# jdhuang-csm/hybrid-drt

Measured on AMD Instinct MI355X. Metric: DRT fits/sec (256 freq x 512 tau, batched), higher is better.
Workload: dtype f64

## Files before the change

hybrid-drt_amd/_ffi.py:

```python
from __future__ import annotations

import ctypes as C
import os
import sys
import threading

import numpy as np

_HERE = os.path.dirname(os.path.abspath(__file__))
LIB_PATH = os.environ.get("HIPDRT_LIB", os.path.join(_HERE, "libhipdrt.so"))

MODE_INTERP, MODE_TRAPZ = 0, 1
RESPONSE_POT, RESPONSE_EXPDECAY = 0, 1
QP_OPTIMAL, QP_MAXITER, QP_SINGULAR_LATE, QP_SINGULAR, QP_ABORTED = 0, 1, 2, -1, -2


class HipDrtError(RuntimeError):
    pass


class QpOpts(C.Structure):
    _fields_ = [("abstol", C.c_double), ("reltol", C.c_double), ("feastol", C.c_double), ("maxiters", C.c_int)]


# ... 44 lines not shown
    "hipdrt_impedance_lookup": [_vp, C.c_double, C.c_int, C.c_int, _dp, _dp, _dp, _dp],
    "hipdrt_impedance_matrix": [_vp, C.c_int, C.c_int, _dp, C.c_int, _dp, C.c_int, C.c_int, C.c_int, C.c_double,
                                C.c_int, _dp, _dp, _dp, _dp, C.c_int, _dp, _dp],
    "hipdrt_impedance_matrix_dev": [_vp, C.c_int, C.c_int, _dp, C.c_int, _dp, C.c_int, C.c_int, C.c_int, C.c_double,
                                    C.c_int, _dp, _dp, _dp, _dp, C.c_int, _vp, _vp, C.c_int, C.POINTER(C.c_float)],
    "hipdrt_phasor_z_matrix": [_vp, _dp, C.c_int, _dp, C.c_int, C.c_double, _dp, _dp],
    "hipdrt_phasor_v_matrix": [_vp, _dp, C.c_int, _dp, C.c_int, C.c_double, _dp, _dp, C.c_int, _dp, _dp],
    "hipdrt_chrono_var_matrix": [_vp, _dp, C.c_int, _ip, C.c_int, C.c_double, C.c_int, _dp],
    "hipdrt_response_lookup": [_vp, C.c_double, C.c_int, C.c_int, _dp, _dp],
    "hipdrt_response_matrix": [_vp, _dp, C.c_int, _dp, C.c_int, _dp, _dp, C.c_int, C.c_int, C.c_double, C.c_int, _dp, _dp,
                               C.c_int, _dp, _dp],
    "hipdrt_plan_bytes_per_spectrum": [C.c_int, C.c_int, C.c_int, C.POINTER(C.c_longlong)],
    "hipdrt_response_matrix_variant": [_vp, _dp, C.c_int, _dp, C.c_int, _dp, _dp, _dp, C.c_int, C.c_int, C.c_double, C.c_int,
                                       _dp, _dp],
    "hipdrt_nonuniform_gaussian_filter1d": [_vp, _dp, C.c_int, _dp, _ip, C.c_int, _ip, _dp, C.c_int, _dp, _dp, C.c_longlong,
                                            _ip, _ip, _dp],
    "hipdrt_penalty_matrices": [_vp, _dp, C.c_int, C.c_double, C.c_int, _dp, _dp, _dp],
    "hipdrt_eis_var_matrix": [_vp, _dp, C.c_int, C.c_double, C.c_double, C.c_int, _dp],
    "hipdrt_qp_batch": [_vp, C.c_int, C.c_int, C.c_int, _dp, _dp, C.c_int, _dp, C.POINTER(QpOpts), _dp, _ip, _dp, _ip],
    "hipdrt_qp_profile": [_vp, C.POINTER(C.c_ulonglong), C.c_int, C.c_int],
    "hipdrt_debug_qp_occupancy": [_vp, C.c_int, C.c_int],
    "hipdrt_debug_qp_group": [_vp, C.c_int],
    "hipdrt_debug_exact_zero_shortcuts": [_vp, C.c_int],
    "hipdrt_debug_qp_waves": [_vp, C.c_int],
    "hipdrt_debug_stream_pool": [_vp, C.c_int, C.POINTER(C.c_void_p), _ip, _ip, _ip],
    "hipdrt_comm_unique_id": [C.c_char_p],
    "hipdrt_comm_create": [C.c_int, C.c_int, C.c_int, C.c_char_p, C.POINTER(_vp)],
    "hipdrt_comm_destroy": [_vp],
    "hipdrt_comm_info": [_vp, _ip, _ip, _ip],
    "hipdrt_comm_broadcast_dev": [_vp, _vp, C.c_longlong, C.c_int],
    "hipdrt_comm_gather_dev": [_vp, _vp, C.c_longlong, _vp, C.c_int],
    "hipdrt_comm_broadcast": [_vp, _dp, C.c_longlong, C.c_int],
    "hipdrt_comm_gather": [_vp, _dp, C.c_longlong, _dp, C.c_int],
    "hipdrt_comm_allreduce_max": [_vp, _dp],
    "hipdrt_comm_barrier": [_vp],
    "hipdrt_device_alloc": [_vp, C.c_longlong, C.POINTER(_vp)],
    "hipdrt_device_free": [_vp, _vp],
    "hipdrt_device_synchronize": [_vp],
    "hipdrt_device_probe": [C.c_int],
    "hipdrt_weighted_gram": [_vp, C.c_int, C.c_int, C.c_int, _dp, _dp, _dp, C.c_int, _dp, _dp, _dp, _dp],
    "hipdrt_default_fit_opts": [C.POINTER(FitOpts)],
    "hipdrt_plan_create": [_vp, _dp, C.c_int, _dp, C.c_int, C.c_double, C.c_int, C.c_int, C.c_int, C.c_int, C.c_int,
                           _dp, _dp, _dp, _dp, C.POINTER(FitOpts), C.c_int, C.POINTER(_vp)],
    "hipdrt_plan_create_prepared": [_vp, C.POINTER(PreparedDesc), _dp, _dp, _dp, _dp, _dp, _dp, _dp, C.POINTER(FitOpts),
                                    C.c_int, C.POINTER(_vp)],
    "hipdrt_plan_upload_prepared": [_vp, C.c_int, C.c_int, _dp, _dp],
# ... 299 lines not shown
        _check(self._lib.hipdrt_device_free(self._h, _vp(ptr)))

    def device_synchronize(self):
        _check(self._lib.hipdrt_device_synchronize(self._h))

    def debug_qp_group(self, members):
        _check(self._lib.hipdrt_debug_qp_group(self._h, int(members)))
        self._qp_group_override = int(members)

    def debug_qp_waves(self, waves):
        _check(self._lib.hipdrt_debug_qp_waves(self._h, int(waves)))

    def debug_stream_pool(self):
        size = C.c_int(0)
        _check(self._lib.hipdrt_debug_stream_pool(self._h, 0, None, None, None, C.byref(size)))
        n = size.value
        st, ho, ru = (C.c_void_p * n)(), (C.c_int * n)(), (C.c_int * n)()
        _check(self._lib.hipdrt_debug_stream_pool(self._h, n, st, ho, ru, C.byref(size)))
        return [st[i] for i in range(n)], [ho[i] for i in range(n)], [ru[i] for i in range(n)]

    def debug_exact_zero_shortcuts(self, on):
        _check(self._lib.hipdrt_debug_exact_zero_shortcuts(self._h, int(bool(on))))

    def qp_profile(self, reset=True):
        buf = (C.c_ulonglong * 64)()
        _check(self._lib.hipdrt_qp_profile(self._h, buf, 64, int(reset)))
        return [int(v) for v in buf]

    def qp_timeline(self):
        n = 64 + 8 * 16 * 8
        buf = (C.c_ulonglong * n)()
        _check(self._lib.hipdrt_qp_profile(self._h, buf, n, 0))
        return np.array(buf[64:], dtype=np.uint64).reshape(8, 16, 8)

    def qp_timeline_mean(self, reset=True):
        nt = 8 * 16 * 8
        n = 64 + 2 * nt + 1
        buf = (C.c_ulonglong * n)()
        _check(self._lib.hipdrt_qp_profile(self._h, buf, n, int(reset)))
        cnt = int(buf[64 + 2 * nt])
        return np.array(buf[64 + nt:64 + 2 * nt], dtype=np.float64).reshape(8, 16, 8) / max(cnt, 1), cnt

    def weighted_gram(self, A, w, b, l2=None, l1=None):
        A, w, b = _f64(A), _f64(w), _f64(b)
        if w.ndim == 1:
            w, b = w[None, :], b[None, :]
# ... 322 lines not shown
```

hybrid-drt_amd/csrc/api.hip:

```cpp
#include <algorithm>
#include <chrono>
#include <cmath>
#include <cstdlib>
#include <cstring>
#include <functional>
#include <memory>
#include <mutex>
#include <new>
#include <stdexcept>

#include "common.hpp"
#include <thread>
#include <vector>

namespace hipdrt {
static thread_local std::string g_err;
void set_error(const std::string& msg) { g_err = msg; }
}

using namespace hipdrt;

struct hipdrt_plan {
    hipdrt_ctx* ctx = nullptr;
    int nf = 0, ntau = 0, n = 0, m = 0, ns = 0, ngrid = 0, ny = 0, mode = 0, toeplitz_a = 0, toeplitz_m = 0;
// ... 246 lines not shown
    hipError_t e = hipGetDeviceCount(&count);
    if (e != hipSuccess || count <= 0) {
        set_error("no HIP device visible (libhipdrt has no CPU fallback)");
        return HIPDRT_E_NODEVICE;
    }
    HIPDRT_REQUIRE(device >= 0 && device < count, "device index out of range");
    HIPDRT_CHECK(hipSetDevice(device)); (void)hipGetLastError();
    hipDeviceProp_t prop;
    HIPDRT_CHECK(hipGetDeviceProperties(&prop, device));
    std::string arch = prop.gcnArchName;
    if (arch.rfind("gfx950", 0) != 0) {
        set_error("device " + std::to_string(device) + " is " + arch + "; libhipdrt is built for gfx950 only");
        return HIPDRT_E_NODEVICE;
    }
    auto* c = new hipdrt_ctx();
    c->device = device;
    c->num_cu = prop.multiProcessorCount;
    c->hbm_bytes = prop.totalGlobalMem;
    c->arch = arch.substr(0, arch.find(':'));
    if (const char* wv = std::getenv("HIPDRT_QP_WAVES")) {
        const int w = std::atoi(wv);
        if (w == 4 || w == 8) c->qp_waves = w;
    }
    if (!pool_hold(c)) { delete c; set_error("no HIP stream could be created on device " + std::to_string(device)); return HIPDRT_E_HIP; }
    *out = c;
    return HIPDRT_OK;
} HIPDRT_CATCH

static std::mutex g_life;

static void free_ctx(hipdrt_ctx* ctx) {
    pool_drop(ctx);
    delete ctx;
}

int hipdrt_destroy(hipdrt_ctx* ctx) try {
    if (!ctx) return HIPDRT_OK;
    std::lock_guard<std::mutex> lk(g_life);
    if (ctx->plans > 0) { ctx->released = true; return HIPDRT_OK; }
    free_ctx(ctx);
    return HIPDRT_OK;
} HIPDRT_CATCH

void* hipdrt_stream(hipdrt_ctx* ctx) { return ctx ? (void*)ctx->stream : nullptr; }

int hipdrt_synchronize(hipdrt_ctx* ctx) try {
// ... 380 lines not shown
    std::lock_guard<std::mutex> lock(pl->mu);
    *size = (int)pl->st.size();
    for (int i = 0; i < std::min(cap, *size); ++i) {
        if (streams) streams[i] = pl->st[i];
        if (holders) holders[i] = pl->holders[i];
        if (running) running[i] = pl->running[i];
    }
    return HIPDRT_OK;
} HIPDRT_CATCH

int hipdrt_debug_qp_waves(hipdrt_ctx* ctx, int waves) try {
    HIPDRT_REQUIRE(ctx, "NULL pointer");
    HIPDRT_REQUIRE(waves == -1 || waves == 4 || waves == 8, "waves: 4, 8 or -1");
    ctx->qp_waves = waves;
    return HIPDRT_OK;
} HIPDRT_CATCH

int hipdrt_debug_exact_zero_shortcuts(hipdrt_ctx* ctx, int on) try {
    HIPDRT_REQUIRE(ctx, "NULL pointer");
    ctx->zero_shortcuts = on ? 1 : 0;
    return HIPDRT_OK;
} HIPDRT_CATCH

int hipdrt_debug_qp_occupancy(hipdrt_ctx* ctx, int threads, int n) try {
    if (!ctx || hipSetDevice(ctx->device) != hipSuccess) return -1;
    return qp_occupancy(threads, n);
} HIPDRT_CATCH

int hipdrt_qp_profile(hipdrt_ctx* ctx, unsigned long long* cycles, int n, int reset) try {
    HIPDRT_REQUIRE(ctx && cycles, "NULL pointer");
    HIPDRT_CHECK(hipSetDevice(ctx->device)); (void)hipGetLastError();
    HIPDRT_CHECK(hipStreamSynchronize(ctx->stream));
    return qp_profile_read(cycles, n, reset) < 0 ? HIPDRT_E_HIP : HIPDRT_OK;
} HIPDRT_CATCH

int hipdrt_weighted_gram(hipdrt_ctx* ctx, int B, int m, int n, const double* A, const double* w, const double* b,
                         int l2_batched, const double* l2, const double* l1, double* P, double* q) try {
    HIPDRT_REQUIRE(ctx && A && w && b && P && q, "NULL pointer");
    HIPDRT_REQUIRE(B >= 1 && m >= 1 && n >= 1, "B, m, n >= 1");
    HIPDRT_CHECK(hipSetDevice(ctx->device)); (void)hipGetLastError();
    hipStream_t st = ctx->stream;
    DevBuf dA, dw, db, dl2, dl1, dP, dq;
    TRY(upload(dA, A, (size_t)m * n * sizeof(double), st));
    TRY(upload(dw, w, (size_t)B * m * sizeof(double), st));
    TRY(upload(db, b, (size_t)B * m * sizeof(double), st));
    if (l2) TRY(upload(dl2, l2, (size_t)(l2_batched ? B : 1) * n * n * sizeof(double), st));
    if (l1) TRY(upload(dl1, l1, (size_t)n * sizeof(double), st));
    HIPDRT_CHECK(dP.alloc((size_t)B * n * n * sizeof(double)));
    HIPDRT_CHECK(dq.alloc((size_t)B * n * sizeof(double)));
    launch_weighted_gram(st, B, m, n, dA.d(), n, dw.d(), db.d(), l2 ? dl2.d() : nullptr,
                         l2_batched ? (long long)n * n : 0, n, l1 ? dl1.d() : nullptr, dP.d(), n, (long long)n * n,
                         dq.d(), nullptr);
    LAUNCH_OK();
    HIPDRT_CHECK(hipMemcpyAsync(P, dP.p, (size_t)B * n * n * sizeof(double), hipMemcpyDeviceToHost, st));
    HIPDRT_CHECK(hipMemcpyAsync(q, dq.p, (size_t)B * n * sizeof(double), hipMemcpyDeviceToHost, st));
    HIPDRT_CHECK(hipStreamSynchronize(st));
    return HIPDRT_OK;
} HIPDRT_CATCH


void hipdrt_default_fit_opts(hipdrt_fit_opts* o) {
    if (!o) return;
    std::memset(o, 0, sizeof(*o));
    o->rp_scale = 14;
    const double dw[3] = {1.5, 1.0, 0.5}, sd[3] = {1, 1000, 1000}, sa[3] = {5, 10, 25}, ra[3] = {0.15, 0.2, 0.25};
    for (int k = 0; k < 3; ++k) {
        o->derivative_weights[k] = dw[k]; o->sigma_ds[k] = sd[k]; o->s_alpha[k] = sa[k]; o->s_0[k] = 1.0;
        o->rho_alpha[k] = ra[k]; o->rho_0[k] = 1.0;
    }
    o->l1_lambda_0 = 0; o->l2_lambda_0 = 142;
    o->iw_l1_lambda_0 = 1e-4; o->iw_l2_lambda_0 = 1e-4;
    o->ohmic_penalty = 1e-6; o->inductance_penalty = 1e-6; o->inductance_scale = 1e-5;
    o->eis_vmm_epsilon = 0.25; o->eis_reim_cor = 0.25;
    o->xtol = 1e-2; o->max_iter = 50; o->nonneg = 1; o->scale_data = 1; o->fit_ohmic = 1; o->fit_inductance = 1;
    o->update_scale = 0; o->eff_hp = 1;
// ... 277 lines not shown
} HIPDRT_CATCH

int hipdrt_plan_upload(hipdrt_plan* p, int B, const double* z_re, const double* z_im) try {
    HIPDRT_REQUIRE(p && z_re && z_im, "NULL pointer");
    HIPDRT_REQUIRE(!p->prepared, "prepared plans take hipdrt_plan_upload_prepared");
    HIPDRT_REQUIRE(B >= 1 && B <= p->capacity, "1 <= B <= capacity");
    HIPDRT_CHECK(hipSetDevice(p->ctx->device)); (void)hipGetLastError();
    hipStream_t st = p->ctx->stream;
    const size_t bytes = (size_t)B * p->nf * sizeof(double);
    HIPDRT_CHECK(hipMemcpyAsync(p->z_re.p, z_re, bytes, hipMemcpyHostToDevice, st));
    HIPDRT_CHECK(hipMemcpyAsync(p->z_im.p, z_im, bytes, hipMemcpyHostToDevice, st));
    HIPDRT_CHECK(hipStreamSynchronize(st));
    p->B = B;
    return HIPDRT_OK;
} HIPDRT_CATCH

static GramL2 plan_l2(const hipdrt_plan* p, double l2_lambda_0, const double* derivative_weights, double dop_l2_lambda_0) {
    GramL2 g{};
    g.l2 = nullptr; g.ldm = p->ldm; g.ns = p->ns; g.use_rho = 1;
    g.sym = p->prepared ? 0 : p->toeplitz_m;
    g.toep = p->toeplitz_m;
    g.toep_maxd = (p->toeplitz_m && !(p->ctx && !p->ctx->zero_shortcuts)) ? p->toep_maxd : -1;
    g.spec_zero = p->spec_zero;
    for (int k = 0; k < 3; ++k) { g.mk[k] = p->mk[k].d(); g.dfac[k] = l2_lambda_0 * derivative_weights[k]; }
    g.s = p->s.d(); g.rho = p->rho.d();
    if (p->prepared && p->desc.dop_size > 0) {
        g.dop_start = p->desc.dop_start; g.dop_size = p->desc.dop_size; g.dop_rho = p->dop_rho.d();
        for (int k = 0; k < 3; ++k) g.dop_dfac[k] = dop_l2_lambda_0 * p->desc.dop_derivative_weights[k];
    }
    return g;
}

struct FinalP { GramL2 g; const double* w; };
static FinalP plan_final_p(const hipdrt_plan* p, int b) {
    FinalP f{plan_l2(p, p->opts.l2_lambda_0, p->opts.derivative_weights, p->prepared ? p->desc.dop_l2_lambda_0 : 0.0),
             p->has_weight_factors() ? p->w_eff.d() : p->w.d()};
    if (b >= 0) {
        f.g.s += (size_t)b * 3 * p->n; f.g.rho += (size_t)b * 3;
        if (f.g.dop_size > 0) f.g.dop_rho += (size_t)b * 3;
        f.w += (size_t)b * p->m;
    }
    return f;
}

static int plan_toep_reach(hipdrt_plan* p) {
    p->toep_maxd = -1;
// ... 221 lines not shown
            launch_scale_rows(st, B, m, p->w.d(), nullptr, 0, p->weight_factor, nullptr, p->w.d());
            launch_scale_rows(st, B, m, p->w.d(), p->wrow.d(), p->wrow_batched, 1.0, nullptr, p->w_eff.d());
        }
        wfin = p->w_eff.d();
    }
    return outer_finish(p, st, tm, wfin);
}

static int subbatch_count(const hipdrt_plan* p) {
    if (p->prepared || p->hist_b >= 0 || p->has_weight_factors() || p->opts.outlier_p > 0.0 || p->qp_G != 0) return 1;
    const int k_auto = p->B >= 1000 ? std::min(4, pool_size(p->ctx->device)) : (p->B >= 600 ? 2 : 1);
    int k = p->subbatches >= 1 ? std::min(p->subbatches, std::max(1, p->B / 64)) : k_auto;
    const int force = p->ctx ? p->ctx->qp_force_group : -1;
    if (qp_group_size(p->B, p->n, force) != 0) return 1;
    while (k > 1 && qp_group_size(p->B / k, p->n, force) != 0) --k;
    return k;
}

static int make_view(hipdrt_plan* p, hipdrt_subfit& sf, int idx, int b0, int nb) {
    hipdrt_plan& v = sf.view;
    sf.ctx.device = p->ctx->device; sf.ctx.num_cu = p->ctx->num_cu; sf.ctx.hbm_bytes = p->ctx->hbm_bytes; sf.ctx.arch = p->ctx->arch;
    sf.ctx.qp_force_group = p->ctx->qp_force_group;
    sf.ctx.zero_shortcuts = p->ctx->zero_shortcuts;
    sf.ctx.qp_waves = p->ctx->qp_waves;
    v.ctx = &sf.ctx;
    v.nf = p->nf; v.ntau = p->ntau; v.n = p->n; v.m = p->m; v.ns = p->ns; v.ngrid = p->ngrid; v.ny = p->ny; v.mode = p->mode;
    v.toeplitz_a = p->toeplitz_a; v.toeplitz_m = p->toeplitz_m; v.toep_maxd = p->toep_maxd; v.spec_zero = p->spec_zero; v.idx_rinf = p->idx_rinf; v.idx_induc = p->idx_induc;
    v.ldrm = p->ldrm; v.ldm = p->ldm; v.ldp = p->ldp; v.ldl = p->ldl; v.eps = p->eps; v.opts = p->opts;
    v.capacity = nb; v.B = nb; v.qp_G = p->qp_G; v.subbatches = 1;
    auto whole = [](DevBuf& d, const DevBuf& s_) { d.alias(s_, 0, s_.bytes); };
    whole(v.freq, p->freq); whole(v.tau, p->tau); whole(v.ln_tau, p->ln_tau); whole(v.wt_re, p->wt_re); whole(v.wt_im, p->wt_im);
    whole(v.lut6, p->lut6); whole(v.a_re, p->a_re); whole(v.a_im, p->a_im); whole(v.cr, p->cr); whole(v.rm, p->rm);
    for (int k = 0; k < 3; ++k) whole(v.mk[k], p->mk[k]);
    whole(v.vmm, p->vmm); whole(v.h, p->h); whole(v.l1, p->l1); whole(v.h_init, p->h_init); whole(v.vmm_base, p->vmm_base);
    whole(v.Ptmp, p->Ptmp);
    const SpecDims d = spec_dims(p);
    for (const PerSpectrumBuf& e : kPerSpectrum) {
        const size_t per = e.bytes(d);
        (v.*e.buf).alias(p->*e.buf, (size_t)b0 * per, (size_t)nb * per);
    }
    v.n_active.alias(p->n_active_sub, (size_t)idx * sizeof(int), sizeof(int));
    return HIPDRT_OK;
}

int hipdrt_plan_bytes_per_spectrum(int nf, int ntau, int ns, long long* bytes) try {
    HIPDRT_REQUIRE(bytes && nf >= 1 && ntau >= 1 && ns >= 0, "arguments");
// ... 443 lines not shown
```

hybrid-drt_amd/csrc/common.hpp:

```cpp
#pragma once
#include <hip/hip_runtime.h>

#include <cstdio>
#include <string>
#include <vector>

#include "../../include/hipdrt.h"
#include "../../include/hipdrt_debug.h"

namespace hipdrt {

void set_error(const std::string& msg);

#define HIPDRT_CHECK(expr)                                                                     \
    do {                                                                                       \
        hipError_t _e = (expr);                                                                \
        if (_e != hipSuccess) {                                                                \
            hipdrt::set_error(std::string(#expr) + ": " + hipGetErrorString(_e) + " (" +       \
                              __FILE__ + ":" + std::to_string(__LINE__) + ")");                \
            return HIPDRT_E_HIP;                                                               \
        }                                                                                      \
    } while (0)

#define HIPDRT_REQUIRE(cond, msg)                                                              \
// ... 40 lines not shown

inline int round_up(int v, int m) { return (v + m - 1) / m * m; }

inline int set_lds_limit(const void* f, size_t bytes, const char* what) {
    const hipError_t e = hipFuncSetAttribute(f, hipFuncAttributeMaxDynamicSharedMemorySize, (int)bytes);
    if (e != hipSuccess) { set_error(std::string("hipFuncSetAttribute(") + what + "): " + hipGetErrorString(e)); return HIPDRT_E_HIP; }
    return HIPDRT_OK;
}

}

struct hipdrt_ctx {
    int device = 0;
    hipStream_t stream = nullptr;
    int pool_idx = -1;
    int num_cu = 0;
    size_t hbm_bytes = 0;
    std::string arch;
    int plans = 0;
    bool released = false;
    int qp_force_group = -1;
    int zero_shortcuts = 1;
    int qp_waves = -1;
};

namespace hipdrt {

void ensure_stream_pool(int device);

void launch_lookup(hipStream_t st, double eps, int ngrid, int ny, const double* wt_re, const double* wt_im,
                   double* z_re, double* z_im);
void launch_lookup_slopes(hipStream_t st, int ngrid, const double* xp, const double* fp, double* slopes);
void launch_impedance_matrix(hipStream_t st, int B, int freq_batched, const double* freq, int nf, const double* tau,
                             int ntau, int mode, int toeplitz, double eps, int ngrid, const double* lut6, int ny,
                             double* a_re, double* a_im, double* cr_scratch);
void launch_phasor_z(hipStream_t st, const double* freq, int nf, const double* nu, int nnu, double eps, double* zre,
                     double* zim);
void launch_phasor_v(hipStream_t st, const double* times, int nt, const double* nu, int nnu, double eps,
                     const double* step_times, const double* step_sizes, int nsteps, double* rm, double* layered);
void launch_chrono_vmm(hipStream_t st, const double* tt, int nt, const int* seg, int nseg, double eps, int uniform,
                       double* vmm);
void launch_response_lookup(hipStream_t st, double eps, int ngrid, int ny, const double* td, double* v);
void launch_response_matrix(hipStream_t st, const double* times, int nt, const double* tau, int ntau,
                            const double* step_times, const double* step_sizes, int nsteps, int mode, double eps,
                            int ngrid, const double* lut3, int ny, double* a, double* layered);
void launch_response_variant(hipStream_t st, const double* times, int nt, const double* tau, int ntau,
// ... 5 lines not shown
void launch_penalty(hipStream_t st, const double* ln_tau, int n, double eps, int toeplitz, double* m0, double* m1,
                    double* m2, int ld, int pad);
void launch_eis_vmm(hipStream_t st, const double* freq, int nf, double vmm_eps, double reim_cor, int uniform,
                    double* vmm);

struct GramL2 {
    const double* l2;
    long long l2_stride;
    int ldl2;
    const double* mk[3];
    int ldm;
    const double* s;
    const double* rho;
    double dfac[3];
    int ns;
    int use_rho;
    int sym;
    int toep;
    int toep_maxd;
    int spec_zero;
    int dop_start, dop_size;
    const double* dop_rho;
    double dop_dfac[3];
};
void launch_gram_l2(hipStream_t st, int B, int m, int n, const double* A, int lda, const double* w, const GramL2& g,
                    double* P, int ldp, long long p_stride, const int* active, double* Ppk = nullptr,
                    long long ppk_stride = 0, int nchp = 0, long long a_stride = 0);
void launch_pack_p(hipStream_t st, int B, int n, const double* P, int ldp, long long p_stride, double* Ppk,
                   long long ppk_stride, int nchp);
inline int qp_nchp(int n) { return round_up(n, 32) / 16; }
inline size_t qp_ppk_doubles(int n) { return (size_t)qp_nchp(n) * qp_nchp(n) * 256; }
void launch_qvec_batched(hipStream_t s, int B, int m, int n, const double* rm, int ldrm, const double* w, const double* y,
                         const double* l1, double l1_scalar, double* q, const int* active);
void launch_qvec(hipStream_t st, int B, int m, int n, const double* A, int lda, const double* w, const double* y,
                 const double* l1, double l1_scalar, double* q, const int* active, long long a_stride = 0);
void launch_weighted_gram(hipStream_t st, int B, int m, int n, const double* A, int lda, const double* w,
                          const double* b, const double* l2, long long l2_stride, int ldl2, const double* l1,
                          double* P, int ldp, long long p_stride, double* q, const int* active);

struct FitState {
    int nf, m, n, ns, ldrm, ldm;
    int toeplitz_m;
    int toep_reach;
    int continue_mode;
    int min_iter;
    double basis_area;
    hipdrt_fit_opts opts;
    int prepared;
    hipdrt_prepared_desc desc;
    long long rm_stride;
    double* rm_rw;
    const double* vz_strength;
    const double* vz_entry;
    double *dop_rho, *dop_xmx;
    double* outlier_t;
    double* hist_dop_rho;
    const double* rm;
    const double* vmm;
    const double* vmm_iw;
    const double* mk[3];
    const double *z_re, *z_im;
// ... 83 lines not shown
```

hybrid-drt_amd/csrc/gram.hip:

```cpp
#include "common.hpp"

namespace hipdrt {

typedef double v4d __attribute__((ext_vector_type(4)));

static constexpr int GT = 64;
static constexpr int GK = 16;
static constexpr int GLD = 80;


template <bool DOP, bool ROWP>
__global__ __launch_bounds__(256, 5) void gram_kernel(int m, int n, const double* __restrict__ A, int lda,
                                                   const double* __restrict__ w, GramL2 g, double* __restrict__ P,
                                                   int ldp, long long p_stride, const int* __restrict__ active,
                                                   int ntile, double* __restrict__ Ppk, long long ppk_stride, int nchp,
                                                   long long a_stride) {
    const int b = blockIdx.y;
    if (active && !active[b]) return;
    A += (size_t)b * a_stride;
    int t = blockIdx.x, ti = 0;
    while (t >= ti + 1) { t -= ti + 1; ++ti; }
    const int tj = t;
    const int i0 = ti * GT, j0 = tj * GT;
    const bool diag = (ti == tj);

    __shared__ double sI[GK * GLD];
    __shared__ double sJ[GK * GLD];

    const int tid = threadIdx.x, lane = tid & 63, wv = tid >> 6;
    const int wi = (wv >> 1) * 32, wj = (wv & 1) * 32;
    const double* wb = w + (size_t)b * m;

    v4d acc[2][2];
#pragma unroll
    for (int a = 0; a < 2; ++a)
#pragma unroll
        for (int c = 0; c < 2; ++c) acc[a][c] = (v4d){0.0, 0.0, 0.0, 0.0};

    const int sk = tid >> 4, sc = (tid & 15) * 4;
    const bool vec2 = ((lda | n) & 1) == 0;
    double vi[4], vj[4], wkr = 0.0;
    auto fetch = [&](int k0) {
        const int k = k0 + sk;
#pragma unroll
        for (int e = 0; e < 4; ++e) { vi[e] = 0.0; vj[e] = 0.0; }
        wkr = 0.0;
        if (k < m) {
            wkr = wb[k];
            const double* row = A + (size_t)k * lda;
            if (vec2) {
#pragma unroll
                for (int e = 0; e < 4; e += 2) {
                    const int ci = i0 + sc + e, cj = j0 + sc + e;
                    if (ci < n) { const double2 t = *reinterpret_cast<const double2*>(row + ci); vi[e] = t.x; vi[e + 1] = t.y; }
                    if (!diag && cj < n) { const double2 t = *reinterpret_cast<const double2*>(row + cj); vj[e] = t.x; vj[e + 1] = t.y; }
                }
            } else {
#pragma unroll
                for (int e = 0; e < 4; ++e) {
                    const int ci = i0 + sc + e, cj = j0 + sc + e;
                    if (ci < n) vi[e] = row[ci];
                    if (!diag && cj < n) vj[e] = row[cj];
                }
            }
        }
    };
    const int nt16 = (n + 15) >> 4;
    const int tr0 = __builtin_amdgcn_readfirstlane((i0 + wi) >> 4), tc0 = __builtin_amdgcn_readfirstlane((j0 + wj) >> 4);
    const bool need00 = tr0 < nt16 && tc0 < nt16 && tr0 >= tc0;
    const bool need01 = tr0 < nt16 && tc0 + 1 < nt16 && tr0 >= tc0 + 1;
    const bool need10 = tr0 + 1 < nt16 && tc0 < nt16 && tr0 + 1 >= tc0;
    const bool need11 = tr0 + 1 < nt16 && tc0 + 1 < nt16 && tr0 + 1 >= tc0 + 1;
    fetch(0);
    for (int k0 = 0; k0 < m; k0 += GK) {
        __syncthreads();
        *reinterpret_cast<double2*>(&sI[sk * GLD + sc]) = make_double2(wkr * vi[0], wkr * vi[1]);
        *reinterpret_cast<double2*>(&sI[sk * GLD + sc + 2]) = make_double2(wkr * vi[2], wkr * vi[3]);
        if (!diag) {
            *reinterpret_cast<double2*>(&sJ[sk * GLD + sc]) = make_double2(wkr * vj[0], wkr * vj[1]);
            *reinterpret_cast<double2*>(&sJ[sk * GLD + sc + 2]) = make_double2(wkr * vj[2], wkr * vj[3]);
        }
        __syncthreads();
        if (k0 + GK < m) fetch(k0 + GK);
        const double* sj = diag ? sI : sJ;
#pragma unroll
        for (int kk = 0; kk < GK; kk += 4) {
            const int kr = kk + (lane >> 4);
            double a0 = sI[kr * GLD + wi + (lane & 15)];
            double a1 = sI[kr * GLD + wi + 16 + (lane & 15)];
            double b0 = sj[kr * GLD + wj + (lane & 15)];
            double b1 = sj[kr * GLD + wj + 16 + (lane & 15)];
            if (need00) acc[0][0] = __builtin_amdgcn_mfma_f64_16x16x4f64(b0, a0, acc[0][0], 0, 0, 0);
            if (need01) acc[0][1] = __builtin_amdgcn_mfma_f64_16x16x4f64(b1, a0, acc[0][1], 0, 0, 0);
            if (need10) acc[1][0] = __builtin_amdgcn_mfma_f64_16x16x4f64(b0, a1, acc[1][0], 0, 0, 0);
            if (need11) acc[1][1] = __builtin_amdgcn_mfma_f64_16x16x4f64(b1, a1, acc[1][1], 0, 0, 0);
        }
    }

    double (*sqI)[GT] = reinterpret_cast<double (*)[GT]>(sI);
    double (*sqJ)[GT] = reinterpret_cast<double (*)[GT]>(sJ);
    constexpr int TW = 2 * GT;
    double (*tw)[TW] = reinterpret_cast<double (*)[TW]>(sI + 3 * GT);
    const int dbase = i0 - j0 - (GT - 1);
    double fac[3] = {0, 0, 0};
    const bool l2on = g.s && !(!DOP && g.toep && g.toep_maxd >= 0 && (j0 >= g.ns || g.spec_zero) && i0 >= g.ns && dbase > g.toep_maxd);
    if (l2on) {
#pragma unroll
        for (int k = 0; k < 3; ++k) fac[k] = g.dfac[k] * (g.use_rho ? g.rho[(size_t)b * 3 + k] : 1.0);
        __syncthreads();
        const double* sb_ = g.s + (size_t)b * 3 * n;
        for (int e = tid; e < 3 * GT; e += 256) {
            const int k = e / GT, c = e % GT;
            sqI[k][c] = (i0 + c < n) ? sqrt(sb_[k * n + i0 + c]) : 0.0;
            sqJ[k][c] = (j0 + c < n) ? sqrt(sb_[k * n + j0 + c]) : 0.0;
        }
        if (g.toep) {
            const int nd = n - g.ns;
            for (int e = tid; e < 3 * TW; e += 256) {
                const int k = e / TW, sl = e % TW;
                int dd = dbase + sl;
                dd = dd < 0 ? -dd : dd;
                tw[k][sl] = (g.dfac[k] > 0.0 && dd < nd) ? g.mk[k][(size_t)g.ns * g.ldm + g.ns + dd] * fac[k] : 0.0;
            }
        }
        __syncthreads();
    }
    double* Pb = (ROWP && P) ? P + (size_t)b * p_stride : nullptr;
    double dfac2[3] = {0, 0, 0};
    if (l2on) {
        if (DOP) {
#pragma unroll
            for (int k = 0; k < 3; ++k) dfac2[k] = g.dop_dfac[k] * (g.use_rho ? g.dop_rho[(size_t)b * 3 + k] : 1.0);
        }
    }
    const int dop_lo = DOP ? g.dop_start : 0, dop_hi = DOP ? g.dop_start + g.dop_size : 0;
    double* Pk = Ppk ? Ppk + (size_t)b * ppk_stride : nullptr;
#pragma unroll
    for (int a = 0; a < 2; ++a)
#pragma unroll
        for (int c = 0; c < 2; ++c) {
            double vals[4];
#pragma unroll
            for (int r = 0; r < 4; ++r) {
                const int i = i0 + wi + a * 16 + (lane & 15);
                const int j = j0 + wj + c * 16 + (lane >> 4) + 4 * r;
                double v = 0.0;
                if (i < n && j < n) {
                    v = acc[a][c][r];
                    if (l2on) {
                        double l2 = 0.0;
#pragma unroll
                        for (int k = 0; k < 3; ++k) {
                            if (g.dfac[k] > 0.0) {
                                double mv;
                                if (g.toep && i >= g.ns && j >= g.ns) {
                                    mv = tw[k][(i - j) - dbase];
                                } else {
                                    mv = g.sym ? g.mk[k][(size_t)j * g.ldm + i] : g.mk[k][(size_t)i * g.ldm + j];
                                    if (i >= g.ns && j >= g.ns) mv *= fac[k];
                                    else if (DOP && i >= dop_lo && i < dop_hi && j >= dop_lo && j < dop_hi) mv *= dfac2[k];
                                }
                                l2 += (sqI[k][i - i0] * mv) * sqJ[k][j - j0];
                            }
                        }
                        v += l2;
                    } else if (!g.s && g.l2) {
                        v += g.l2[(size_t)b * g.l2_stride + (size_t)i * g.ldl2 + j];
                    }
                    if (ROWP && Pb && !(diag && j > i)) {
                        Pb[(size_t)i * ldp + j] = v;
                        if (i != j) Pb[(size_t)j * ldp + i] = v;
                    }
                }
                vals[r] = v;
            }
            if (Pk) {
                const int tr = ((i0 + wi) >> 4) + a, tc = ((j0 + wj) >> 4) + c;
                if (tr < nchp && tc < nchp && tr >= tc) {
                    double2* tile = reinterpret_cast<double2*>(Pk + ((size_t)tr * nchp + tc) * 256);
                    const int fo = (lane & 15) * 4 + (lane >> 4);
                    tile[fo] = make_double2(vals[0], vals[1]);
                    tile[64 + fo] = make_double2(vals[2], vals[3]);
                }
            }
        }
}

__global__ __launch_bounds__(64) void pack_p_kernel(int n, const double* __restrict__ P, int ldp, long long p_stride,
                                                    double* __restrict__ Ppk, long long ppk_stride, int nchp) {
    int t = blockIdx.x, tr = 0;
    while (t >= tr + 1) { t -= tr + 1; ++tr; }
    const int tc = t, b = blockIdx.y, lane = threadIdx.x;
    const double* Pb = P + (size_t)b * p_stride;
    double vals[4];
#pragma unroll
    for (int r = 0; r < 4; ++r) {
        const int i = tr * 16 + (lane & 15), j = tc * 16 + (lane >> 4) + 4 * r;
        double v = 0.0;
        if (i < n && j < n) v = (i >= j) ? Pb[(size_t)i * ldp + j] : Pb[(size_t)j * ldp + i];
        vals[r] = v;
    }
    double2* tile = reinterpret_cast<double2*>(Ppk + (size_t)b * ppk_stride + ((size_t)tr * nchp + tc) * 256);
    const int fo = (lane & 15) * 4 + (lane >> 4);
// ... 65 lines not shown
        __syncthreads();
    }
    const int r = ti * 16 + i, cc = tj * 16 + j;
    if (r < nrow && cc < nrow) {
        out[(size_t)r * ld + cc] = acc * scale;
        out[(size_t)cc * ld + r] = acc * scale;
    }
}

void launch_rows_outer(hipStream_t st, const double* Y, int nch, int ncol, int nex, int nrow, double scale, double* out, int ld) {
    hipLaunchKernelGGL(rows_outer_kernel, dim3(nex, nex), dim3(256), 0, st, Y, nch, ncol, nrow, scale, out, ld);
}

void launch_pack_p(hipStream_t st, int B, int n, const double* P, int ldp, long long p_stride, double* Ppk,
                   long long ppk_stride, int nchp) {
    const int nt = (n + 15) / 16;
    hipLaunchKernelGGL(pack_p_kernel, dim3(nt * (nt + 1) / 2, B), dim3(64), 0, st, n, P, ldp, p_stride, Ppk, ppk_stride,
                       nchp);
}

void launch_gram_l2(hipStream_t st, int B, int m, int n, const double* A, int lda, const double* w, const GramL2& g,
                    double* P, int ldp, long long p_stride, const int* active, double* Ppk, long long ppk_stride,
                    int nchp, long long a_stride) {
    const int nt = (n + GT - 1) / GT;
    const int ntile = nt * (nt + 1) / 2;
    const bool dop = g.s && g.dop_size > 0;
#define HIPDRT_GRAM(D, R) hipLaunchKernelGGL((gram_kernel<D, R>), dim3(ntile, B), dim3(256), 0, st, m, n, A, lda, w, g, P, ldp, \
                                             p_stride, active, ntile, Ppk, ppk_stride, nchp, a_stride)
    if (P) { if (dop) HIPDRT_GRAM(true, true); else HIPDRT_GRAM(false, true); }
    else { if (dop) HIPDRT_GRAM(true, false); else HIPDRT_GRAM(false, false); }
#undef HIPDRT_GRAM
}

void launch_qvec(hipStream_t st, int B, int m, int n, const double* A, int lda, const double* w, const double* y,
                 const double* l1, double l1_scalar, double* q, const int* active, long long a_stride) {
    if (a_stride == 0 && (size_t)m * n < ((size_t)1 << 20)) {
        launch_qvec_batched(st, B, m, n, A, lda, w, y, l1, l1_scalar, q, active);
        return;
    }
    hipLaunchKernelGGL(qvec_kernel, dim3((n + 255) / 256, B), dim3(256), 0, st, m, n, A, lda, w, y, l1, l1_scalar, q,
                       active, a_stride);
}

void launch_weighted_gram(hipStream_t st, int B, int m, int n, const double* A, int lda, const double* w,
                          const double* b, const double* l2, long long l2_stride, int ldl2, const double* l1,
                          double* P, int ldp, long long p_stride, double* q, const int* active) {
    GramL2 g{};
    g.l2 = l2; g.l2_stride = l2_stride; g.ldl2 = ldl2; g.s = nullptr;
    launch_gram_l2(st, B, m, n, A, lda, w, g, P, ldp, p_stride, active);
    launch_qvec(st, B, m, n, A, lda, w, b, l1, 0.0, q, active);
}

}
```

include/hipdrt_debug.h:

```cpp
#ifndef HIPDRT_DEBUG_H
#define HIPDRT_DEBUG_H

#include "hipdrt.h"

#ifdef __cplusplus
extern "C" {
#endif

int hipdrt_qp_profile(hipdrt_ctx* ctx, unsigned long long* cycles, int n, int reset);
int hipdrt_debug_qp_occupancy(hipdrt_ctx* ctx, int threads, int n);
int hipdrt_debug_qp_group(hipdrt_ctx* ctx, int members);
int hipdrt_debug_qp_waves(hipdrt_ctx* ctx, int waves);
int hipdrt_debug_exact_zero_shortcuts(hipdrt_ctx* ctx, int on);
int hipdrt_debug_stream_pool(hipdrt_ctx* ctx, int cap, void** streams, int* holders, int* running, int* size);

#ifdef __cplusplus
}
#endif

#endif
```

Measured before the change: 2666.

## Fold trailing 16-column Gram strip into diagonal tiles to drop a tile row

When n leaves exactly one 16-wide column chunk past a multiple of 64, the Gram kernel no longer launches an extra row of 64x64 tiles. Instead each diagonal block computes that leftover strip: one wave does the strip-times-tile products and the corner wave adds the strip's self-product, with separate L2 penalty tables staged in shared memory. The global loads are also rewritten with scalar base pointers and 32-bit byte offsets, so n is capped at 2^23. This cuts launched blocks and wasted MFMA work on mostly empty edge tiles, at the cost of extra load imbalance on the diagonal blocks and more complex indexing.

Result: faster. 2725, median of 6 (+2.2%).

```diff
diff --git a/hybrid-drt_amd/_ffi.py b/hybrid-drt_amd/_ffi.py
--- a/hybrid-drt_amd/_ffi.py
+++ b/hybrid-drt_amd/_ffi.py
@@ -90,6 +90,7 @@
     "hipdrt_debug_qp_occupancy": [_vp, C.c_int, C.c_int],
     "hipdrt_debug_qp_group": [_vp, C.c_int],
     "hipdrt_debug_exact_zero_shortcuts": [_vp, C.c_int],
+    "hipdrt_debug_gram_fold": [_vp, C.c_int],
     "hipdrt_debug_qp_waves": [_vp, C.c_int],
     "hipdrt_debug_stream_pool": [_vp, C.c_int, C.POINTER(C.c_void_p), _ip, _ip, _ip],
     "hipdrt_comm_unique_id": [C.c_char_p],
@@ -435,6 +436,9 @@
     def debug_exact_zero_shortcuts(self, on):
         _check(self._lib.hipdrt_debug_exact_zero_shortcuts(self._h, int(bool(on))))
 
+    def debug_gram_fold(self, on):
+        _check(self._lib.hipdrt_debug_gram_fold(self._h, int(bool(on))))
+
     def qp_profile(self, reset=True):
         buf = (C.c_ulonglong * 64)()
         _check(self._lib.hipdrt_qp_profile(self._h, buf, 64, int(reset)))
diff --git a/hybrid-drt_amd/csrc/api.hip b/hybrid-drt_amd/csrc/api.hip
--- a/hybrid-drt_amd/csrc/api.hip
+++ b/hybrid-drt_amd/csrc/api.hip
@@ -292,6 +292,7 @@
         const int w = std::atoi(wv);
         if (w == 4 || w == 8) c->qp_waves = w;
     }
+    if (const char* gf = std::getenv("HIPDRT_GRAM_FOLD")) c->gram_fold = std::atoi(gf) != 0;
     if (!pool_hold(c)) { delete c; set_error("no HIP stream could be created on device " + std::to_string(device)); return HIPDRT_E_HIP; }
     *out = c;
     return HIPDRT_OK;
@@ -718,6 +719,12 @@
     return HIPDRT_OK;
 } HIPDRT_CATCH
 
+int hipdrt_debug_gram_fold(hipdrt_ctx* ctx, int on) try {
+    HIPDRT_REQUIRE(ctx, "NULL pointer");
+    ctx->gram_fold = on ? 1 : 0;
+    return HIPDRT_OK;
+} HIPDRT_CATCH
+
 int hipdrt_debug_qp_occupancy(hipdrt_ctx* ctx, int threads, int n) try {
     if (!ctx || hipSetDevice(ctx->device) != hipSuccess) return -1;
     return qp_occupancy(threads, n);
@@ -734,6 +741,7 @@
                          int l2_batched, const double* l2, const double* l1, double* P, double* q) try {
     HIPDRT_REQUIRE(ctx && A && w && b && P && q, "NULL pointer");
     HIPDRT_REQUIRE(B >= 1 && m >= 1 && n >= 1, "B, m, n >= 1");
+    HIPDRT_REQUIRE(n <= GRAM_MAX_LD, "n <= 2^23 (the Gram kernel's 32-bit slab offsets)");
     HIPDRT_CHECK(hipSetDevice(ctx->device)); (void)hipGetLastError();
     hipStream_t st = ctx->stream;
     DevBuf dA, dw, db, dl2, dl1, dP, dq;
@@ -746,7 +754,7 @@
     HIPDRT_CHECK(dq.alloc((size_t)B * n * sizeof(double)));
     launch_weighted_gram(st, B, m, n, dA.d(), n, dw.d(), db.d(), l2 ? dl2.d() : nullptr,
                          l2_batched ? (long long)n * n : 0, n, l1 ? dl1.d() : nullptr, dP.d(), n, (long long)n * n,
-                         dq.d(), nullptr);
+                         dq.d(), nullptr, !ctx->gram_fold);
     LAUNCH_OK();
     HIPDRT_CHECK(hipMemcpyAsync(P, dP.p, (size_t)B * n * n * sizeof(double), hipMemcpyDeviceToHost, st));
     HIPDRT_CHECK(hipMemcpyAsync(q, dq.p, (size_t)B * n * sizeof(double), hipMemcpyDeviceToHost, st));
@@ -1070,6 +1078,7 @@
     g.toep = p->toeplitz_m;
     g.toep_maxd = (p->toeplitz_m && !(p->ctx && !p->ctx->zero_shortcuts)) ? p->toep_maxd : -1;
     g.spec_zero = p->spec_zero;
+    g.no_fold = p->ctx && !p->ctx->gram_fold;
     for (int k = 0; k < 3; ++k) { g.mk[k] = p->mk[k].d(); g.dfac[k] = l2_lambda_0 * derivative_weights[k]; }
     g.s = p->s.d(); g.rho = p->rho.d();
     if (p->prepared && p->desc.dop_size > 0) {
@@ -1337,6 +1346,7 @@
     sf.ctx.device = p->ctx->device; sf.ctx.num_cu = p->ctx->num_cu; sf.ctx.hbm_bytes = p->ctx->hbm_bytes; sf.ctx.arch = p->ctx->arch;
     sf.ctx.qp_force_group = p->ctx->qp_force_group;
     sf.ctx.zero_shortcuts = p->ctx->zero_shortcuts;
+    sf.ctx.gram_fold = p->ctx->gram_fold;
     sf.ctx.qp_waves = p->ctx->qp_waves;
     v.ctx = &sf.ctx;
     v.nf = p->nf; v.ntau = p->ntau; v.n = p->n; v.m = p->m; v.ns = p->ns; v.ngrid = p->ngrid; v.ny = p->ny; v.mode = p->mode;
diff --git a/hybrid-drt_amd/csrc/common.hpp b/hybrid-drt_amd/csrc/common.hpp
--- a/hybrid-drt_amd/csrc/common.hpp
+++ b/hybrid-drt_amd/csrc/common.hpp
@@ -86,6 +86,7 @@
     int qp_force_group = -1;
     int zero_shortcuts = 1;
     int qp_waves = -1;
+    int gram_fold = 1;
 };
 
 namespace hipdrt {
@@ -137,7 +138,9 @@
     int dop_start, dop_size;
     const double* dop_rho;
     double dop_dfac[3];
-};
+    int no_fold;
+};
+constexpr int GRAM_MAX_LD = 1 << 23;
 void launch_gram_l2(hipStream_t st, int B, int m, int n, const double* A, int lda, const double* w, const GramL2& g,
                     double* P, int ldp, long long p_stride, const int* active, double* Ppk = nullptr,
                     long long ppk_stride = 0, int nchp = 0, long long a_stride = 0);
@@ -151,7 +154,7 @@
                  const double* l1, double l1_scalar, double* q, const int* active, long long a_stride = 0);
 void launch_weighted_gram(hipStream_t st, int B, int m, int n, const double* A, int lda, const double* w,
                           const double* b, const double* l2, long long l2_stride, int ldl2, const double* l1,
-                          double* P, int ldp, long long p_stride, double* q, const int* active);
+                          double* P, int ldp, long long p_stride, double* q, const int* active, int no_fold = 0);
 
 struct FitState {
     int nf, m, n, ns, ldrm, ldm;
diff --git a/hybrid-drt_amd/csrc/gram.hip b/hybrid-drt_amd/csrc/gram.hip
--- a/hybrid-drt_amd/csrc/gram.hip
+++ b/hybrid-drt_amd/csrc/gram.hip
@@ -1,8 +1,15 @@
+#include <cassert>
+#include <type_traits>
+
 #include "common.hpp"
 
 namespace hipdrt {
 
 typedef double v4d __attribute__((ext_vector_type(4)));
+typedef const __attribute__((address_space(1))) char* gbytes;
+typedef const __attribute__((address_space(1))) double* gdouble;
+typedef double v2d __attribute__((ext_vector_type(2)));
+typedef const __attribute__((address_space(1))) v2d* gdouble2;
 
 static constexpr int GT = 64;
 static constexpr int GK = 16;
@@ -13,7 +20,7 @@
 __global__ __launch_bounds__(256, 5) void gram_kernel(int m, int n, const double* __restrict__ A, int lda,
                                                    const double* __restrict__ w, GramL2 g, double* __restrict__ P,
                                                    int ldp, long long p_stride, const int* __restrict__ active,
-                                                   int ntile, double* __restrict__ Ppk, long long ppk_stride, int nchp,
+                                                   int fold, double* __restrict__ Ppk, long long ppk_stride, int nchp,
                                                    long long a_stride) {
     const int b = blockIdx.y;
     if (active && !active[b]) return;
@@ -27,9 +34,14 @@
     __shared__ double sI[GK * GLD];
     __shared__ double sJ[GK * GLD];
 
-    const int tid = threadIdx.x, lane = tid & 63, wv = tid >> 6;
+    const int tid = threadIdx.x, lane = tid & 63, wv = __builtin_amdgcn_readfirstlane(tid >> 6);
     const int wi = (wv >> 1) * 32, wj = (wv & 1) * 32;
-    const double* wb = w + (size_t)b * m;
+
+    const int nt16 = (n + 15) >> 4;
+    const int is0 = (nt16 - 1) * 16;
+    const bool fstrip = fold && diag;
+    const bool stripw = fstrip && wv == 1;
+    const bool corner = fstrip && wv == 0 && i0 + GT == is0;
 
     v4d acc[2][2];
 #pragma unroll
@@ -37,92 +49,160 @@
 #pragma unroll
         for (int c = 0; c < 2; ++c) acc[a][c] = (v4d){0.0, 0.0, 0.0, 0.0};
 
-    const int sk = tid >> 4, sc = (tid & 15) * 4;
+    const int sk = tid >> 4, sc = (tid & 15) * 4, scol = is0 + (tid & 15);
     const bool vec2 = ((lda | n) & 1) == 0;
+#define HIPDRT_SCALAR_BASE(p_) asm volatile("" : "+s"(p_))
+#define HIPDRT_VECTOR_OFFSETS() asm volatile("" : "+v"(oi), "+v"(oj), "+v"(os), "+v"(ow))
     double vi[4], vj[4], wkr = 0.0;
-    auto fetch = [&](int k0) {
-        const int k = k0 + sk;
+    gbytes ap = (gbytes)A;
+    gbytes wp = (gbytes)(w + (size_t)b * m);
+    unsigned oi = (unsigned)(sk * lda + i0 + sc) * 8u, oj = (unsigned)(sk * lda + j0 + sc) * 8u;
+    unsigned os = (unsigned)(sk * lda + scol) * 8u, ow = (unsigned)sk * 8u;
+    const bool sv = fstrip && scol < n;
+    auto fetch = [&](int k0, auto diag_tag) {
+        constexpr bool DG = decltype(diag_tag)::value;
+        HIPDRT_SCALAR_BASE(ap); HIPDRT_SCALAR_BASE(wp); HIPDRT_VECTOR_OFFSETS();
 #pragma unroll
         for (int e = 0; e < 4; ++e) { vi[e] = 0.0; vj[e] = 0.0; }
         wkr = 0.0;
-        if (k < m) {
-            wkr = wb[k];
-            const double* row = A + (size_t)k * lda;
+        if (k0 + sk < m) {
+            wkr = *(gdouble)(wp + ow);
             if (vec2) {
 #pragma unroll
                 for (int e = 0; e < 4; e += 2) {
                     const int ci = i0 + sc + e, cj = j0 + sc + e;
-                    if (ci < n) { const double2 t = *reinterpret_cast<const double2*>(row + ci); vi[e] = t.x; vi[e + 1] = t.y; }
-                    if (!diag && cj < n) { const double2 t = *reinterpret_cast<const double2*>(row + cj); vj[e] = t.x; vj[e + 1] = t.y; }
+                    if (ci < n) { const v2d t = *(gdouble2)(ap + oi + e * 8); vi[e] = t.x; vi[e + 1] = t.y; }
+                    if (!DG && cj < n) { const v2d t = *(gdouble2)(ap + oj + e * 8); vj[e] = t.x; vj[e + 1] = t.y; }
                 }
             } else {
 #pragma unroll
                 for (int e = 0; e < 4; ++e) {
                     const int ci = i0 + sc + e, cj = j0 + sc + e;
-                    if (ci < n) vi[e] = row[ci];
-                    if (!diag && cj < n) vj[e] = row[cj];
-                }
-            }
-        }
+                    if (ci < n) vi[e] = *(gdouble)(ap + oi + e * 8);
+                    if (!DG && cj < n) vj[e] = *(gdouble)(ap + oj + e * 8);
+                }
+            }
+            if (DG && sv) vj[0] = *(gdouble)(ap + os);
+        }
+        ap += (size_t)GK * lda * sizeof(double);
+        wp += GK * sizeof(double);
     };
-    const int nt16 = (n + 15) >> 4;
-    const int tr0 = __builtin_amdgcn_readfirstlane((i0 + wi) >> 4), tc0 = __builtin_amdgcn_readfirstlane((j0 + wj) >> 4);
+#undef HIPDRT_SCALAR_BASE
+#undef HIPDRT_VECTOR_OFFSETS
+    const int tr0 = (i0 + wi) >> 4, tc0 = (j0 + wj) >> 4;
     const bool need00 = tr0 < nt16 && tc0 < nt16 && tr0 >= tc0;
     const bool need01 = tr0 < nt16 && tc0 + 1 < nt16 && tr0 >= tc0 + 1;
     const bool need10 = tr0 + 1 < nt16 && tc0 < nt16 && tr0 + 1 >= tc0;
     const bool need11 = tr0 + 1 < nt16 && tc0 + 1 < nt16 && tr0 + 1 >= tc0 + 1;
-    fetch(0);
-    for (int k0 = 0; k0 < m; k0 += GK) {
-        __syncthreads();
-        *reinterpret_cast<double2*>(&sI[sk * GLD + sc]) = make_double2(wkr * vi[0], wkr * vi[1]);
-        *reinterpret_cast<double2*>(&sI[sk * GLD + sc + 2]) = make_double2(wkr * vi[2], wkr * vi[3]);
-        if (!diag) {
-            *reinterpret_cast<double2*>(&sJ[sk * GLD + sc]) = make_double2(wkr * vj[0], wkr * vj[1]);
-            *reinterpret_cast<double2*>(&sJ[sk * GLD + sc + 2]) = make_double2(wkr * vj[2], wkr * vj[3]);
-        }
-        __syncthreads();
-        if (k0 + GK < m) fetch(k0 + GK);
-        const double* sj = diag ? sI : sJ;
-#pragma unroll
-        for (int kk = 0; kk < GK; kk += 4) {
-            const int kr = kk + (lane >> 4);
-            double a0 = sI[kr * GLD + wi + (lane & 15)];
-            double a1 = sI[kr * GLD + wi + 16 + (lane & 15)];
-            double b0 = sj[kr * GLD + wj + (lane & 15)];
-            double b1 = sj[kr * GLD + wj + 16 + (lane & 15)];
-            if (need00) acc[0][0] = __builtin_amdgcn_mfma_f64_16x16x4f64(b0, a0, acc[0][0], 0, 0, 0);
-            if (need01) acc[0][1] = __builtin_amdgcn_mfma_f64_16x16x4f64(b1, a0, acc[0][1], 0, 0, 0);
-            if (need10) acc[1][0] = __builtin_amdgcn_mfma_f64_16x16x4f64(b0, a1, acc[1][0], 0, 0, 0);
-            if (need11) acc[1][1] = __builtin_amdgcn_mfma_f64_16x16x4f64(b1, a1, acc[1][1], 0, 0, 0);
-        }
-    }
+    auto kloop = [&](auto&& fetch_next, auto mode_tag) {
+        constexpr int MODE = decltype(mode_tag)::value;
+        constexpr std::bool_constant<MODE != 0> DG{};
+        fetch_next(0, DG);
+        for (int k0 = 0; k0 < m; k0 += GK) {
+            __syncthreads();
+            *reinterpret_cast<double2*>(&sI[sk * GLD + sc]) = make_double2(wkr * vi[0], wkr * vi[1]);
+            *reinterpret_cast<double2*>(&sI[sk * GLD + sc + 2]) = make_double2(wkr * vi[2], wkr * vi[3]);
+            if (MODE == 0) {
+                *reinterpret_cast<double2*>(&sJ[sk * GLD + sc]) = make_double2(wkr * vj[0], wkr * vj[1]);
+                *reinterpret_cast<double2*>(&sJ[sk * GLD + sc + 2]) = make_double2(wkr * vj[2], wkr * vj[3]);
+            } else if (MODE == 2 || fstrip) {
+                sI[sk * GLD + GT + (tid & 15)] = wkr * vj[0];
+            }
+            __syncthreads();
+            if (k0 + GK < m) fetch_next(k0 + GK, DG);
+            if constexpr (MODE == 2) {
+#pragma unroll
+                for (int kk = 0; kk < GK; kk += 4) {
+                    const int kr = kk + (lane >> 4);
+                    double as = sI[kr * GLD + GT + (lane & 15)];
+                    double b0 = sI[kr * GLD + (lane & 15)];
+                    double b1 = sI[kr * GLD + 16 + (lane & 15)];
+                    double b2 = sI[kr * GLD + 32 + (lane & 15)];
+                    double b3 = sI[kr * GLD + 48 + (lane & 15)];
+                    acc[0][0] = __builtin_amdgcn_mfma_f64_16x16x4f64(b0, as, acc[0][0], 0, 0, 0);
+                    acc[0][1] = __builtin_amdgcn_mfma_f64_16x16x4f64(b1, as, acc[0][1], 0, 0, 0);
+                    acc[1][0] = __builtin_amdgcn_mfma_f64_16x16x4f64(b2, as, acc[1][0], 0, 0, 0);
+                    acc[1][1] = __builtin_amdgcn_mfma_f64_16x16x4f64(b3, as, acc[1][1], 0, 0, 0);
+                }
+            } else {
+                const double* sj = MODE == 1 ? sI : sJ;
+#pragma unroll
+                for (int kk = 0; kk < GK; kk += 4) {
+                    const int kr = kk + (lane >> 4);
+                    double a0 = sI[kr * GLD + wi + (lane & 15)];
+                    double a1 = sI[kr * GLD + wi + 16 + (lane & 15)];
+                    double b0 = sj[kr * GLD + wj + (lane & 15)];
+                    double b1 = sj[kr * GLD + wj + 16 + (lane & 15)];
+                    if (need00) acc[0][0] = __builtin_amdgcn_mfma_f64_16x16x4f64(b0, a0, acc[0][0], 0, 0, 0);
+                    if (need01) acc[0][1] = __builtin_amdgcn_mfma_f64_16x16x4f64(b1, a0, acc[0][1], 0, 0, 0);
+                    if (need10) acc[1][0] = __builtin_amdgcn_mfma_f64_16x16x4f64(b0, a1, acc[1][0], 0, 0, 0);
+                    if (need11) acc[1][1] = __builtin_amdgcn_mfma_f64_16x16x4f64(b1, a1, acc[1][1], 0, 0, 0);
+                    if (MODE == 1 && corner) {
+                        double as = sI[kr * GLD + GT + (lane & 15)];
+                        acc[0][1] = __builtin_amdgcn_mfma_f64_16x16x4f64(as, as, acc[0][1], 0, 0, 0);
+                    }
+                }
+            }
+        }
+    };
+    auto kloops = [&](auto&& fetch_next) {
+        if (!diag) kloop(fetch_next, std::integral_constant<int, 0>{});
+        else if (!stripw) kloop(fetch_next, std::integral_constant<int, 1>{});
+        else kloop(fetch_next, std::integral_constant<int, 2>{});
+    };
+#pragma unroll
+    for (int e = 0; e < 4; ++e) vj[e] = 0.0;
+    kloops(fetch);
+
+    int tid_e = tid;
+    asm volatile("" : "+v"(tid_e));
+    const int lane_e = tid_e & 63;
 
     double (*sqI)[GT] = reinterpret_cast<double (*)[GT]>(sI);
     double (*sqJ)[GT] = reinterpret_cast<double (*)[GT]>(sJ);
     constexpr int TW = 2 * GT;
     double (*tw)[TW] = reinterpret_cast<double (*)[TW]>(sI + 3 * GT);
     const int dbase = i0 - j0 - (GT - 1);
+    constexpr int SW = GT + 16;
+    constexpr int SQS = 3 * GT + 3 * TW, TWS = SQS + 3 * 16;
+    static_assert(TWS + 3 * SW <= GK * GLD, "the strip's tables fit behind the tile's");
+    const int dbase_s = is0 - j0 - (GT - 1);
     double fac[3] = {0, 0, 0};
     const bool l2on = g.s && !(!DOP && g.toep && g.toep_maxd >= 0 && (j0 >= g.ns || g.spec_zero) && i0 >= g.ns && dbase > g.toep_maxd);
+    const bool l2on_s = g.s && !(!DOP && g.toep && g.toep_maxd >= 0 && (j0 >= g.ns || g.spec_zero) && is0 >= g.ns && dbase_s > g.toep_maxd);
     if (l2on) {
 #pragma unroll
         for (int k = 0; k < 3; ++k) fac[k] = g.dfac[k] * (g.use_rho ? g.rho[(size_t)b * 3 + k] : 1.0);
         __syncthreads();
         const double* sb_ = g.s + (size_t)b * 3 * n;
-        for (int e = tid; e < 3 * GT; e += 256) {
+        for (int e = tid_e; e < 3 * GT; e += 256) {
             const int k = e / GT, c = e % GT;
             sqI[k][c] = (i0 + c < n) ? sqrt(sb_[k * n + i0 + c]) : 0.0;
             sqJ[k][c] = (j0 + c < n) ? sqrt(sb_[k * n + j0 + c]) : 0.0;
         }
+        const int nd = n - g.ns;
         if (g.toep) {
-            const int nd = n - g.ns;
-            for (int e = tid; e < 3 * TW; e += 256) {
+            for (int e = tid_e; e < 3 * TW; e += 256) {
                 const int k = e / TW, sl = e % TW;
                 int dd = dbase + sl;
                 dd = dd < 0 ? -dd : dd;
                 tw[k][sl] = (g.dfac[k] > 0.0 && dd < nd) ? g.mk[k][(size_t)g.ns * g.ldm + g.ns + dd] * fac[k] : 0.0;
             }
         }
+        if (fstrip) {
+            if (tid_e < 3 * 16) {
+                const int k = tid_e / 16, c = tid_e % 16;
+                sI[SQS + tid_e] = (is0 + c < n) ? sqrt(sb_[k * n + is0 + c]) : 0.0;
+            }
+            if (g.toep && l2on_s) {
+                for (int e = tid_e; e < 3 * SW; e += 256) {
+                    const int k = e / SW, sl = e % SW;
+                    int dd = dbase_s + sl;
+                    dd = dd < 0 ? -dd : dd;
+                    sI[TWS + e] = (g.dfac[k] > 0.0 && dd < nd) ? g.mk[k][(size_t)g.ns * g.ldm + g.ns + dd] * fac[k] : 0.0;
+                }
+            }
+        }
         __syncthreads();
     }
     double* Pb = (ROWP && P) ? P + (size_t)b * p_stride : nullptr;
@@ -139,28 +219,39 @@
     for (int a = 0; a < 2; ++a)
 #pragma unroll
         for (int c = 0; c < 2; ++c) {
+            int ib = i0 + wi + a * 16, jb = j0 + wj + c * 16, rs = GT, cs = GT, ws = TW, db = dbase;
+            const double *rt = sI + wi + a * 16, *ct = sJ + wj + c * 16, *wt = sI + 3 * GT;
+            bool l2sub = l2on;
+            if (stripw) {
+                ib = is0; jb = j0 + (2 * a + c) * 16;
+                rt = sI + SQS; rs = 16; ct = sJ + (2 * a + c) * 16;
+                wt = sI + TWS; ws = SW; db = dbase_s; l2sub = l2on_s;
+            } else if (corner && a == 0 && c == 1) {
+                ib = jb = is0;
+                rt = ct = sI + SQS; rs = cs = 16;
+            }
             double vals[4];
 #pragma unroll
             for (int r = 0; r < 4; ++r) {
-                const int i = i0 + wi + a * 16 + (lane & 15);
-                const int j = j0 + wj + c * 16 + (lane >> 4) + 4 * r;
+                const int i = ib + (lane_e & 15);
+                const int j = jb + (lane_e >> 4) + 4 * r;
                 double v = 0.0;
                 if (i < n && j < n) {
                     v = acc[a][c][r];
-                    if (l2on) {
+                    if (l2sub) {
                         double l2 = 0.0;
 #pragma unroll
                         for (int k = 0; k < 3; ++k) {
                             if (g.dfac[k] > 0.0) {
                                 double mv;
                                 if (g.toep && i >= g.ns && j >= g.ns) {
-                                    mv = tw[k][(i - j) - dbase];
+                                    mv = wt[k * ws + (i - j) - db];
                                 } else {
                                     mv = g.sym ? g.mk[k][(size_t)j * g.ldm + i] : g.mk[k][(size_t)i * g.ldm + j];
                                     if (i >= g.ns && j >= g.ns) mv *= fac[k];
                                     else if (DOP && i >= dop_lo && i < dop_hi && j >= dop_lo && j < dop_hi) mv *= dfac2[k];
                                 }
-                                l2 += (sqI[k][i - i0] * mv) * sqJ[k][j - j0];
+                                l2 += (rt[k * rs + (i - ib)] * mv) * ct[k * cs + (j - jb)];
                             }
                         }
                         v += l2;
@@ -175,10 +266,10 @@
                 vals[r] = v;
             }
             if (Pk) {
-                const int tr = ((i0 + wi) >> 4) + a, tc = ((j0 + wj) >> 4) + c;
+                const int tr = ib >> 4, tc = jb >> 4;
                 if (tr < nchp && tc < nchp && tr >= tc) {
                     double2* tile = reinterpret_cast<double2*>(Pk + ((size_t)tr * nchp + tc) * 256);
-                    const int fo = (lane & 15) * 4 + (lane >> 4);
+                    const int fo = (lane_e & 15) * 4 + (lane_e >> 4);
                     tile[fo] = make_double2(vals[0], vals[1]);
                     tile[64 + fo] = make_double2(vals[2], vals[3]);
                 }
@@ -290,11 +381,14 @@
 void launch_gram_l2(hipStream_t st, int B, int m, int n, const double* A, int lda, const double* w, const GramL2& g,
                     double* P, int ldp, long long p_stride, const int* active, double* Ppk, long long ppk_stride,
                     int nchp, long long a_stride) {
-    const int nt = (n + GT - 1) / GT;
-    const int ntile = nt * (nt + 1) / 2;
+    assert(n <= lda && lda <= GRAM_MAX_LD);
+    const int nt = (n + GT - 1) / GT, nt16 = (n + 15) / 16;
+    const int fold = !g.no_fold && nt >= 2 && nt16 - 4 * (nt - 1) == 1;
+    const int ntr = fold ? nt - 1 : nt;
+    const int ntile = ntr * (ntr + 1) / 2;
     const bool dop = g.s && g.dop_size > 0;
 #define HIPDRT_GRAM(D, R) hipLaunchKernelGGL((gram_kernel<D, R>), dim3(ntile, B), dim3(256), 0, st, m, n, A, lda, w, g, P, ldp, \
-                                             p_stride, active, ntile, Ppk, ppk_stride, nchp, a_stride)
+                                             p_stride, active, fold, Ppk, ppk_stride, nchp, a_stride)
     if (P) { if (dop) HIPDRT_GRAM(true, true); else HIPDRT_GRAM(false, true); }
     else { if (dop) HIPDRT_GRAM(true, false); else HIPDRT_GRAM(false, false); }
 #undef HIPDRT_GRAM
@@ -312,9 +406,9 @@
 
 void launch_weighted_gram(hipStream_t st, int B, int m, int n, const double* A, int lda, const double* w,
                           const double* b, const double* l2, long long l2_stride, int ldl2, const double* l1,
-                          double* P, int ldp, long long p_stride, double* q, const int* active) {
+                          double* P, int ldp, long long p_stride, double* q, const int* active, int no_fold) {
     GramL2 g{};
-    g.l2 = l2; g.l2_stride = l2_stride; g.ldl2 = ldl2; g.s = nullptr;
+    g.l2 = l2; g.l2_stride = l2_stride; g.ldl2 = ldl2; g.s = nullptr; g.no_fold = no_fold;
     launch_gram_l2(st, B, m, n, A, lda, w, g, P, ldp, p_stride, active);
     launch_qvec(st, B, m, n, A, lda, w, b, l1, 0.0, q, active);
 }
diff --git a/include/hipdrt_debug.h b/include/hipdrt_debug.h
--- a/include/hipdrt_debug.h
+++ b/include/hipdrt_debug.h
@@ -12,6 +12,7 @@
 int hipdrt_debug_qp_group(hipdrt_ctx* ctx, int members);
 int hipdrt_debug_qp_waves(hipdrt_ctx* ctx, int waves);
 int hipdrt_debug_exact_zero_shortcuts(hipdrt_ctx* ctx, int on);
+int hipdrt_debug_gram_fold(hipdrt_ctx* ctx, int on);
 int hipdrt_debug_stream_pool(hipdrt_ctx* ctx, int cap, void** streams, int* holders, int* running, int* size);
 
 #ifdef __cplusplus
```
